# JianCao92/speaker-diarization

Measured on AMD Instinct MI355X. Metric: diarized audio throughput (CD gw/BIC + CL hi/BIC), higher is better.
Workload: dtype f64

## Files before the change

speaker-diarization_amd/csrc/spkd_cluster.hpp:

```cpp
#pragma once
#include "spkd_device.hpp"
#include "spkd_quad.hpp"
#include "spkd_tri.hpp"
#include "../../include/spkd.h"

namespace spkd {

constexpr double MAXINT_F = 9223372036854775808.0;
constexpr double PEN_UNIT = 39.0 + 0.5 * 39.0 * 40.0;
constexpr int AUX = 3 * DA;
constexpr int ERR_DEGENERATE_MERGE = 2;

__device__ __forceinline__ unsigned long long dkey(double v) {
    unsigned long long b = (unsigned long long)__double_as_longlong(v);
    b = (b << 1) ? b : 0ull;
    return (b >> 63) ? ~b : (b | 0x8000000000000000ull);
}
__device__ __forceinline__ double dkey_inv(unsigned long long k) {
    unsigned long long b = (k >> 63) ? (k & 0x7fffffffffffffffull) : ~k;
    return __longlong_as_double((long long)b);
}
template <bool MAXOP>
__device__ __forceinline__ unsigned wave_red_u32(unsigned x) {
    auto op = [](unsigned a, unsigned b) { return MAXOP ? (a > b ? a : b) : (a < b ? a : b); };
// ... 389 lines not shown
    int64_t c = w * 4 + L.m;
    const bool valid = c < n_rec;
    c = valid ? c : n_rec - 1;
    const double* R = qr + c * QREC;
    QuadRows q;
    double sv[QS];
    const double nR = qr_count(R), fR = fast_recip(nR - 1.0);
    quad_load_scaled(R, L.t, fR, q, sv);
    double c1[QS];
    const double gR = -(fR * fast_recip(nR));
#pragma unroll
    for (int s = 0; s < QS; ++s) c1[s] = gR * sv[s];
    TriRank1<0>::run(q, c1, sv);
    auto form_single = [&](int mi, double (&a)[DA]) { single_pair_matrix(kind, recs[mi], recs[mi], true, a); };
    const double v = tri_logdet(q, L.m, err, form_single);
    if (valid && L.t == 0) ld[c] = v;
}

__global__ __launch_bounds__(PT_WAVES * WAVE) void k_cluster_prep(
        const double* __restrict__ qr, int64_t n_rec, int kind,
        double* __restrict__ ld, double* __restrict__ aux, int* err,
        double* pinv_ws) {
    cluster_prep_block(qr, n_rec, kind, ld, aux, err, pinv_ws, blockIdx.x);
}

__global__ __launch_bounds__(PT_WAVES * WAVE) void k_cluster_prep_batch(
        const double* __restrict__ qr, const int64_t* __restrict__ seg_off, int kind,
        double* __restrict__ ld, double* __restrict__ aux, int* prob_err,
        double* pinv_ws) {
    const int64_t off = seg_off[blockIdx.x];
    cluster_prep_block(qr + off * QREC, seg_off[blockIdx.x + 1] - off, kind, ld + off, aux + off * AUX,
                       prob_err + blockIdx.x, pinv_ws, blockIdx.y);
}

__device__ __forceinline__ double finish_distance(int kind, double lambdac, double nA, double ldA,
                                                  double nC, double ldC, double ldx) {
#pragma clang fp contract(off)
    const double n = nA + nC;
    if (kind == SPKD_BIC) {
        double d = 0.5 * n * ldx - 0.5 * nA * ldA - 0.5 * nC * ldC;
        d -= lambdac * 0.5 * PEN_UNIT * log(n);
        return d;
    }
    return -(n / 2.0) * ((nA / n) * ldA + (nC / n) * ldC - ldx);
}

__device__ __forceinline__ int find_problem(const int64_t* __restrict__ seg_off, int64_t n_prob, int64_t g) {
    int64_t lo = 0, hi = n_prob;
    while (hi - lo > 1) {
        int64_t mid = (lo + hi) >> 1;
        if (seg_off[mid] <= g) lo = mid; else hi = mid;
    }
    return (int)lo;
}

#ifndef SPKD_MX_WAVES
#define SPKD_MX_WAVES 4
#endif
constexpr int MX_WAVES = SPKD_MX_WAVES;

template <bool TWO>
__global__ __launch_bounds__(MX_WAVES * WAVE, 2) void k_matrix(
        const double* __restrict__ ex, const double* __restrict__ pk, const int64_t* __restrict__ seg_off,
        const int32_t* __restrict__ rec_prob, const int32_t* __restrict__ sched, int variant, int kind, double lambdac,
        const double* __restrict__ ld, const double* __restrict__ aux,
        double* __restrict__ mat, const int64_t* __restrict__ mat_off,
        unsigned long long* stat_max, unsigned long long* stat_min, int* err) {
    __shared__ double ldsA[QREC];
    const int64_t g = sched[blockIdx.x];
    if (g < 0) return;
    const int p = rec_prob[g];
    const int64_t off = seg_off[p];
    const int64_t N = seg_off[p + 1] - off;
    const int64_t ra = g - off;
    double* Dm = mat + mat_off[p];
    const double* A = ex + g * QREC;
    stage_record(ldsA, A, threadIdx.x, MX_WAVES * WAVE);
    if (variant == 1) {
        if (threadIdx.x == 0) Dm[ra * N + ra] = MAXINT_F;
    } else {
        for (int64_t c = threadIdx.x; c <= ra; c += MX_WAVES * WAVE) Dm[ra * N + c] = __builtin_huge_val();
    }
    __syncthreads();
    const double nA = ldsA[QREC_COUNT_AT];
    const double ldA = ld[g];
    const int wave = threadIdx.x >> 6;
    const QuadLane L = quad_lane();
    if (kind == SPKD_KL2) {
        double wmax = __builtin_nan(""), wmin = __builtin_nan("");
        for (int64_t rc = ra + 1 + wave; rc < N; rc += MX_WAVES) {
            const double d = kl2_from_aux(aux + g * AUX, aux + (off + rc) * AUX);
            if (lane_id() == 0) {
                Dm[ra * N + rc] = d;
                if (variant == 1) Dm[rc * N + ra] = d;
            }
            if (stat_valid(d)) {
                wmax = (wmax != wmax || d > wmax) ? d : wmax;
                wmin = (wmin != wmin || d < wmin) ? d : wmin;
            }
        }
        if (variant == 1 && lane_id() == 0) {
            if (wmax == wmax) atomicMax(stat_max + p, dkey(wmax));
            if (wmin == wmin) atomicMin(stat_min + p, dkey(wmin));
        }
        return;
    }
    double* row = Dm + ra * N;
    for (int64_t base = ra + 1 + 4 * wave; base < N; base += 4 * MX_WAVES) {
        int64_t rc = base + L.m;
        const bool valid = rc < N;
        rc = valid ? rc : N - 1;
        const double det = quad_pair_det<TWO>(kind, ldsA, nA, A, ex + (off + rc) * QREC, pk + (off + rc) * REC, false, L, err);
        if (valid && L.t == 0) row[rc] = det;
    }
    __syncthreads();
    double wmax = __builtin_nan(""), wmin = __builtin_nan("");
    for (int64_t c = ra + 1 + threadIdx.x; c < N; c += MX_WAVES * WAVE) {
        const double det = row[c];
        const double nC = pk[(off + c) * REC + REC - 1];
        const double d = finish_distance(kind, lambdac, nA, ldA, nC, ld[off + c], log(det));
        row[c] = d;
        if (variant == 1) {
            Dm[c * N + ra] = d;
            if (stat_valid(d)) {
                wmax = (wmax != wmax || d > wmax) ? d : wmax;
                wmin = (wmin != wmin || d < wmin) ? d : wmin;
            }
        }
    }
    if (variant == 1) {
        const unsigned long long kmax = wave_red_u64<true>(wmax == wmax ? dkey(wmax) : 0ull);
        const unsigned long long kmin = wave_red_u64<false>(wmin == wmin ? dkey(wmin) : ~0ull);
        if (lane_id() == 0) {
            if (kmax != 0ull) atomicMax(stat_max + p, kmax);
            if (kmin != ~0ull) atomicMin(stat_min + p, kmin);
        }
    }
}

constexpr int AHC_WAVES = 8;
constexpr int AHC_TPB = AHC_WAVES * WAVE;

#ifdef SPKD_PROFILE
__device__ unsigned long long g_step_prof[8];
__device__ unsigned long long g_ahc_prof[8];
constexpr int AHC_SPAN_PROBS = 4096;
__device__ unsigned long long g_ahc_span[2 * AHC_SPAN_PROBS];
#endif
constexpr int NO_COL = 0x7fffffff;
constexpr int AHC_MAX_N = 65536;


struct RowMin { double mv; int mc, nc; };

template <class Alive>
__device__ __forceinline__ RowMin scan_row(const double* __restrict__ row, long long N, Alive alive,
                                           long long sub_col, double sub_val, int lane) {
    double mv = __builtin_huge_val();
    int mc = NO_COL, nc = NO_COL;
    for (long long c0 = 0; c0 < N; c0 += 4 * WAVE) {
        double v[4];
        int a[4];
#pragma unroll
        for (int u = 0; u < 4; ++u) {
            const long long c = c0 + u * WAVE + lane;
            const long long cc = c < N ? c : N - 1;
            a[u] = (c < N) ? (alive(cc) ? 1 : 0) : 0;
            v[u] = row[cc];
        }
#pragma unroll
        for (int u = 0; u < 4; ++u) {
            const long long cl = c0 + u * WAVE + lane;
            const int c = (int)cl;
            if (!a[u]) continue;
            const double x = (cl == sub_col) ? sub_val : v[u];
            if (x != x) { if (c < nc) nc = c; continue; }
            if (x < mv || (x == mv && c < mc)) { mv = x; mc = c; }
        }
    }
    unsigned long long okey;
    unsigned oc;
    wave_argmin_key(mc != NO_COL ? dkey(mv) : ~0ull, (unsigned)mc, okey, oc);
    RowMin r;
    r.mv = okey != ~0ull ? dkey_inv(okey) : __builtin_huge_val();
    r.mc = okey != ~0ull ? (int)oc : NO_COL;
    r.nc = __any(nc != NO_COL) ? (int)wave_red_u32<false>((unsigned)nc) : NO_COL;
    return r;
}

__device__ __forceinline__ bool row_cache_after_merge(int variant, double d, int sa, int sb,
                                                      double& rm, int& ra, int& rn) {
    if (variant != 1) return ra == sb || rn == sb;
    const bool nan_hit = rn == sa || rn == sb;
    if (ra == sa || ra == sb || nan_hit) {
        if (nan_hit || !(d < rm)) return true;
        rm = d; ra = sa;
    } else if (d != d) {
        if (sa < rn) rn = sa;
    } else if (d < rm || (d == rm && sa < ra)) {
        rm = d; ra = sa;
    }
    return false;
}

template <class Alive>
__device__ __forceinline__ double final_matrix_max(const double* __restrict__ Dm, long long N, Alive alive,
                                                   double* s_tmax, int tid) {
    const int lane = tid & (WAVE - 1), wave = tid >> 6;
    double tmax = -__builtin_huge_val();
    bool anynan = false;
    for (long long r = wave; r < N; r += AHC_WAVES) {
        if (!alive(r)) continue;
        const double* row = Dm + r * N;
        for (long long c = lane; c < N; c += WAVE) {
            if (!alive(c)) continue;
            const double v = row[c];
            if (v != v) anynan = true; else tmax = v > tmax ? v : tmax;
        }
    }
#pragma unroll
    for (int s = 1; s < WAVE; s <<= 1) {
        const double t2 = __shfl_xor(tmax, s);
        tmax = t2 > tmax ? t2 : tmax;
    }
    anynan = __any(anynan);
    if (lane == 0) s_tmax[wave] = anynan ? __builtin_nan("") : tmax;
    __syncthreads();
    double mx = s_tmax[0];
    if (tid == 0) {
        for (int w = 1; w < AHC_WAVES; ++w) {
            const double x = s_tmax[w];
            if (mx == mx) mx = (x != x) ? x : (x > mx ? x : mx);
        }
    }
    return mx;
}

__device__ __forceinline__ void refresh_rows(const double* __restrict__ Dm, long long N,
                                             const int32_t* __restrict__ al, int32_t* __restrict__ dirty,
                                             double* __restrict__ rmin, int32_t* __restrict__ rarg,
                                             int32_t* __restrict__ rnan, unsigned long long* masks,
                                             int tid, int wave, int lane) {
    const long long n_chunks = (N + WAVE - 1) / WAVE;
    for (long long ch = wave; ch < n_chunks; ch += AHC_WAVES) {
        const long long rl = ch * WAVE + lane;
        const long long rc = rl < N ? rl : N - 1;
        const int fa = al[rc], fd = dirty[rc];
        const unsigned long long mk = __ballot(rl < N && fa && fd);
        if (lane == 0) masks[ch] = mk;
    }
    __syncthreads();
    int ord = 0;
    for (long long ch = 0; ch < n_chunks; ++ch) {
        const long long r0 = ch * WAVE;
        unsigned long long todo = masks[ch];
        while (todo) {
            const int b = __builtin_ctzll(todo);
            todo &= todo - 1;
            if ((ord++ & (AHC_WAVES - 1)) != wave) continue;
            const long long r = r0 + b;
            const RowMin e = scan_row(Dm + r * N, N, [&](long long c) { return al[c] != 0; }, -1, 0.0, lane);
            if (lane == 0) { rmin[r] = e.mv; rarg[r] = e.mc; rnan[r] = e.nc; dirty[r] = 0; }
#ifdef SPKD_PROFILE
            if (lane == 0) atomicAdd(&g_ahc_prof[0], 1ull);
#endif
        }
    }
}

template <bool TWO>
__global__ __launch_bounds__(AHC_TPB) void k_ahc(
        double* __restrict__ ex, double* __restrict__ pk, const int64_t* __restrict__ seg_off,
        int variant, int kind, int max_spk, double lambdac, double threshold,
        double* __restrict__ ld, double* __restrict__ aux,
        double* __restrict__ mat, const int64_t* __restrict__ mat_off,
        int32_t* __restrict__ alive, double* __restrict__ tmp,
        double* __restrict__ rmin_all, int32_t* __restrict__ rcache_all,
        int32_t* __restrict__ out_n, int32_t* __restrict__ out_a, int32_t* __restrict__ out_b,
        double* __restrict__ out_d, unsigned long long* stat_max, unsigned long long* stat_min,
        double* __restrict__ final_max, double* __restrict__ final_min, int* err,
        double* pinv_ws, const int32_t* __restrict__ prob_of_block) {
    extern __shared__ int32_t ids[];
    __shared__ double ldsA[QREC];
    __shared__ unsigned long long red3[AHC_WAVES][3];
    __shared__ unsigned long long s_masks[AHC_MAX_N / WAVE];
    __shared__ int s_cnt[2];
    __shared__ int s_nids;
    __shared__ int s_next;
    __shared__ double s_tmax[AHC_WAVES];
    const int tid = threadIdx.x, lane = lane_id(), wave = tid >> 6;
    const QuadLane L = quad_lane();
    const int p = prob_of_block ? prob_of_block[blockIdx.x] : (int)blockIdx.x;
#ifdef SPKD_PROFILE
    if (tid == 0 && p < AHC_SPAN_PROBS) g_ahc_span[2 * p] = wall_clock64();
#endif
    const int64_t off = seg_off[p];
    const long long N = seg_off[p + 1] - off;
    double* Dm = mat + mat_off[p];
    int32_t* al = alive + off;
    double* ldp = ld + off;
    double* tp = tmp + off;
    double* rmin = rmin_all + off;
    int32_t* rarg = rcache_all + 3 * off;
    int32_t* rnan = rarg + N;
    int32_t* dirty = rnan + N;
    for (long long c = tid; c < N; c += AHC_TPB) { al[c] = 1; dirty[c] = 1; }
    __syncthreads();
    long long m = N;
    int n_merges = 0;
    const long long INF_IDX = 0x7fffffffffffffffLL;
    double fmin = 0.0;
#ifdef SPKD_PROFILE
    unsigned long long ahc_acc[5] = {0ull, 0ull, 0ull, 0ull, 0ull}, ahc_t = clock64();
#define AHC_TICK(i) do { const unsigned long long now_ = clock64(); ahc_acc[i] += now_ - ahc_t; ahc_t = now_; } while (0)
#else
#define AHC_TICK(i) ((void)0)
#endif
    while (true) {
        refresh_rows(Dm, N, al, dirty, rmin, rarg, rnan, s_masks, tid, wave, lane);
        __syncthreads();
        AHC_TICK(0);
        unsigned long long kb = ~0ull, ib = ~0ull, inan = ~0ull;
        for (long long r = tid; r < N; r += AHC_TPB) {
            if (!al[r]) continue;
            const double v = rmin[r];
            const int c = rarg[r], nc = rnan[r];
            if (nc != NO_COL) { const unsigned long long l = (unsigned long long)(r * N + nc); inan = l < inan ? l : inan; }
            if (c != NO_COL) {
                const unsigned long long kv = dkey(v);
                if (kv < kb) { kb = kv; ib = (unsigned long long)(r * N + c); }
            }
        }
        {
            const unsigned long long wk = wave_red_u64<false>(kb);
            const unsigned long long wi = wave_red_u64<false>(kb == wk ? ib : ~0ull);
            const unsigned long long wn = __any(inan != ~0ull) ? wave_red_u64<false>(inan) : ~0ull;
            if (lane == 0) { red3[wave][0] = wk; red3[wave][1] = wi; red3[wave][2] = wn; }
        }
        __syncthreads();
        unsigned long long bk = red3[0][0], bi = red3[0][1], bn = red3[0][2];
#pragma unroll
        for (int w = 1; w < AHC_WAVES; ++w) {
            const unsigned long long ok = red3[w][0], oi = red3[w][1], on = red3[w][2];
            const bool t = ok < bk || (ok == bk && oi < bi);
            bk = t ? ok : bk; bi = t ? oi : bi;
            bn = on < bn ? on : bn;
        }
        const bool has_nan = bn != ~0ull;
        const double mind = has_nan ? __builtin_nan("") : (bi != ~0ull ? dkey_inv(bk) : __builtin_huge_val());
        const long long index = has_nan ? (long long)bn : (bi != ~0ull ? (long long)bi : INF_IDX);
        fmin = mind;
        const bool go = (mind <= threshold) || (max_spk > 0 && m > max_spk);
        if (!go) break;
        AHC_TICK(1);
        const long long r0 = index / N, c0 = index - r0 * N;
        if (r0 == c0) {
            if (tid == 0) atomicOr(err, ERR_DEGENERATE_MERGE);
            break;
        }
        const long long sa = r0 < c0 ? r0 : c0, sb = r0 < c0 ? c0 : r0;
        if (tid < 2) s_cnt[tid] = 0;
        if (tid == 0) { s_nids = 1; s_next = 0; }
        __syncthreads();
        {
            int ca = 0, cb = 0;
            for (long long c = tid; c < sb; c += AHC_TPB) {
                if (al[c]) { cb++; if (c < sa) ca++; }
            }
            ca = __builtin_amdgcn_readlane(wave_scan_i32(ca), WAVE - 1);
            cb = __builtin_amdgcn_readlane(wave_scan_i32(cb), WAVE - 1);
            if (lane == 0 && ca) atomicAdd(&s_cnt[0], ca);
            if (lane == 0 && cb) atomicAdd(&s_cnt[1], cb);
        }
        __syncthreads();
        if (tid == 0) {
            const int64_t o = off + n_merges;
            out_a[o] = s_cnt[0]; out_b[o] = s_cnt[1]; out_d[o] = mind;
            al[sb] = 0;
            ids[0] = (int32_t)sa;
        }
        n_merges++;
        m--;
#ifdef SPKD_PROFILE
        if (tid == 0) atomicAdd(&g_ahc_prof[1], 1ull);
#endif
        double* A = ex + (off + sa) * QREC;
        const double* B = ex + (off + sb) * QREC;
        {
            double* Ap = pk + (off + sa) * REC;
            const double* Bp = pk + (off + sb) * REC;
            constexpr int NQ = (QREC + AHC_TPB - 1) / AHC_TPB, NP = (REC + AHC_TPB - 1) / AHC_TPB;
            double qa[NQ], qb[NQ], pa[NP], pb[NP];
#pragma unroll
            for (int u = 0; u < NQ; ++u) {
                const int e = tid + u * AHC_TPB;
                qa[u] = A[e < QREC ? e : 0]; qb[u] = B[e < QREC ? e : 0];
            }
#pragma unroll
            for (int u = 0; u < NP; ++u) {
                const int e = tid + u * AHC_TPB;
                pa[u] = Ap[e < REC ? e : 0]; pb[u] = Bp[e < REC ? e : 0];
            }
#pragma unroll
            for (int u = 0; u < NQ; ++u) {
                const int e = tid + u * AHC_TPB;
                const double v = qa[u] + qb[u];
                if (e < QREC) { A[e] = v; ldsA[e] = v; }
            }
#pragma unroll
            for (int u = 0; u < NP; ++u) {
                const int e = tid + u * AHC_TPB;
                if (e < REC) Ap[e] = pa[u] + pb[u];
            }
        }
        __syncthreads();
        for (long long c0 = 0; c0 < N; c0 += AHC_TPB) {
            const long long c = c0 + tid;
            const bool take = c < N && c != sa && al[c < N ? c : N - 1];
            const unsigned long long mk = __ballot(take);
            int base = 0;
            if (lane == 0 && mk) base = atomicAdd(&s_nids, __popcll(mk));
            base = __shfl(base, 0);
            if (take) ids[base + __popcll(mk & ((1ull << lane) - 1ull))] = (int32_t)c;
        }
        __syncthreads();
        AHC_TICK(2);
        const int nids = s_nids;
        const double nA = ldsA[QREC_COUNT_AT];
        if (kind == SPKD_KL2) {
            if (wave == 0) kl2_aux_from_qr(ldsA, aux + (off + sa) * AUX, pinv_ws);
        } else {
            for (;;) {
                int q4 = 0;
                if (lane == 0) q4 = atomicAdd(&s_next, 1);
                const int base = 4 * __builtin_amdgcn_readfirstlane(q4);
                if (base >= nids) break;
                int k = base + L.m;
                const bool valid = k < nids;
                k = valid ? k : nids - 1;
                const int32_t slot = ids[k];
                const double v = quad_pair_det<TWO>(kind, ldsA, nA, A, ex + (off + slot) * QREC, pk + (off + slot) * REC, k == 0, L, err);
                if (valid && L.t == 0) {
                    if (k == 0) ldp[sa] = log(v); else tp[slot] = v;
                }
            }
        }
        __syncthreads();
        AHC_TICK(3);
        double wmax = __builtin_nan(""), wmin = __builtin_nan("");
        const double ldA = ldp[sa];
        for (long long c = tid; c < N; c += AHC_TPB) {
            if (c == sa || !al[c]) continue;
            double d;
            if (kind == SPKD_KL2) {
                d = kl2_from_aux_serial(aux + (off + sa) * AUX, aux + (off + c) * AUX);
            } else {
                const double nC = qr_count(ex + (off + c) * QREC);
                d = finish_distance(kind, lambdac, nA, ldA, nC, ldp[c], log(tp[c]));
            }
            Dm[sa * N + c] = d;
            const double rm0 = rmin[c];
            const int ra0 = rarg[c], rn0 = rnan[c];
            double rm = rm0;
            int ra = ra0, rn = rn0;
            if (variant == 1) Dm[c * N + sa] = d;
            if (row_cache_after_merge(variant, d, (int)sa, (int)sb, rm, ra, rn)) dirty[c] = 1;
            else {
                if (rm != rm0 || ra != ra0) { rmin[c] = rm; rarg[c] = ra; }
                if (rn != rn0) rnan[c] = rn;
            }
            if (variant == 1 && stat_valid(d)) {
                wmax = (wmax != wmax || d > wmax) ? d : wmax;
                wmin = (wmin != wmin || d < wmin) ? d : wmin;
            }
        }
        if (tid == 0) dirty[sa] = 1;
        if (variant == 1) {
            const unsigned long long kmax = wave_red_u64<true>(wmax == wmax ? dkey(wmax) : 0ull);
            const unsigned long long kmin = wave_red_u64<false>(wmin == wmin ? dkey(wmin) : ~0ull);
            if (lane == 0) {
                if (kmax != 0ull) atomicMax(stat_max + p, kmax);
                if (kmin != ~0ull) atomicMin(stat_min + p, kmin);
            }
        }
        __syncthreads();
        AHC_TICK(4);
    }
#ifdef SPKD_PROFILE
    if (tid == 0) for (int i = 0; i < 5; ++i) atomicAdd(&g_ahc_prof[2 + i], ahc_acc[i]);
#endif
    const double mx = final_matrix_max(Dm, N, [&](long long c) { return al[c] != 0; }, s_tmax, tid);
    if (tid == 0) {
        out_n[p] = n_merges;
        final_max[p] = mx;
        final_min[p] = fmin;
#ifdef SPKD_PROFILE
        if (p < AHC_SPAN_PROBS) g_ahc_span[2 * p + 1] = wall_clock64();
#endif
    }
}

constexpr int STEP_WAVES = 4;
constexpr int STEP_WIDE_FROM = 1024;
constexpr int STEP_PARTNERS = 4 * STEP_WAVES - 1;
constexpr int ALIVE_ROUND = 0x7fffffff;
constexpr int STEP_MAX_N = 16384;
constexpr int STEP_IDX_SHIFT = 14;

struct StepState {
    int32_t done, n_merges;
    long long psa;
    double fmin;
    double diag;
};

__host__ __device__ inline unsigned long long step_slot_word(int round, int new_slot, int old_slot) {
    return ((unsigned long long)(unsigned)round << 40) | ((unsigned long long)(unsigned)new_slot << 20) |
           (unsigned long long)(unsigned)old_slot;
}
__device__ __forceinline__ int step_slot_of(unsigned long long w, int k) {
    return ((int)(w >> 40) < k) ? (int)((w >> 20) & 0xfffffull) : (int)(w & 0xfffffull);
}

struct StepSel {
    double rmin, newrow;
    int32_t rarg, rnan, death, pad;
};

struct StepArrays {
    double* ex;
    double* pk;
    double* exm;
    double* pkm;
    int32_t* death;
    StepSel* sel2;
    unsigned long long* sw;
    double* cnt;
    StepState* state2;
    int64_t n_total;
    int32_t n_prob;
};

__global__ __launch_bounds__(AHC_TPB) void k_step_init(
        const int64_t* __restrict__ seg_off, const double* __restrict__ mat,
        const int64_t* __restrict__ mat_off, StepArrays Q) {
    const int lane = lane_id(), wave = threadIdx.x >> 6;
    const int p = blockIdx.y;
    const int64_t off = seg_off[p];
    const long long N = seg_off[p + 1] - off;
    if (blockIdx.x == 0 && threadIdx.x == 0) {
        StepState S;
        S.done = 0; S.n_merges = 0; S.psa = -1; S.fmin = 0.0; S.diag = 0.0;
        Q.state2[(size_t)1 * Q.n_prob + p] = S;
        Q.state2[(size_t)0 * Q.n_prob + p] = S;
    }
    const long long r = (long long)blockIdx.x * AHC_WAVES + wave;
    if (r >= N) return;
    const RowMin m = scan_row(mat + mat_off[p] + r * N, N, [](long long) { return true; }, -1, 0.0, lane);
    if (lane == 0) {
        StepSel e;
        e.rmin = m.mv; e.newrow = 0.0; e.rarg = m.mc; e.rnan = m.nc; e.death = ALIVE_ROUND; e.pad = 0;
        Q.sel2[Q.n_total + off + r] = e;
        Q.sel2[off + r] = e;
        Q.death[off + r] = ALIVE_ROUND;
        Q.sw[off + r] = step_slot_word(0, (int)r, (int)r);
        Q.cnt[off + r] = Q.pk[(off + r) * REC + REC - 1];
    }
}

template <bool TWO, int SW, int SP>
__global__ __launch_bounds__(SW * WAVE) void k_ahc_step(
        int k, const int64_t* __restrict__ seg_off, int variant, int kind, int max_spk, double lambdac,
        double threshold, double* __restrict__ ld, double* __restrict__ aux,
        double* __restrict__ mat, const int64_t* __restrict__ mat_off, StepArrays Q,
        int32_t* __restrict__ out_a, int32_t* __restrict__ out_b, double* __restrict__ out_d,
        unsigned long long* stat_max, unsigned long long* stat_min, int* err,
        double* pinv_ws) {
    constexpr int TPB = SW * WAVE;
    extern __shared__ int32_t s_dyn[];
    __shared__ double ldsA[QREC];
    __shared__ double s_auxA[AUX];
    __shared__ double s_ldx[4 * STEP_WAVES];
    __shared__ double s_dfin[4 * STEP_WAVES];
    __shared__ int s_rescan[4 * STEP_WAVES];
    struct WaveRed { unsigned long long kb, kr, kmax, kmin; unsigned ib, inan; int mc, nc; };
    __shared__ WaveRed wred[SW];
    __shared__ int s_cnt[2];
    const int tid = threadIdx.x, lane = lane_id(), wave = tid >> 6;
    const QuadLane L = quad_lane();
    const int p = blockIdx.y;
#ifdef SPKD_PROFILE
    unsigned long long st_t = clock64();
#define STEP_TICK(i) do { const unsigned long long now_ = clock64(); if (blockIdx.x == 0 && tid == 0) atomicAdd(&g_ahc_prof[i], now_ - st_t); st_t = now_; } while (0)
    unsigned long long st_f = st_t;
#define STEP_FINE(i) do { const unsigned long long now_ = clock64(); if (blockIdx.x == 0 && tid == 0) atomicAdd(&g_step_prof[i], now_ - st_f); st_f = now_; } while (0)
#else
#define STEP_TICK(i) ((void)0)
#define STEP_FINE(i) ((void)0)
#endif
    asm volatile("" :: "s"(Q.state2), "s"(Q.sel2), "s"(Q.sw), "s"(Q.ex), "s"(Q.exm), "s"(Q.n_total), "s"(Q.n_prob),
                 "s"(seg_off), "s"(mat_off), "s"(mat), "s"(k));
    StepState S = Q.state2[(size_t)(k & 1) * Q.n_prob + p];
    StepState* Snext = Q.state2 + (size_t)((k + 1) & 1) * Q.n_prob + p;
    int64_t off = seg_off[p], off_end = seg_off[p + 1], moff = mat_off[p];
    asm volatile("" :: "s"(S.done), "s"(S.n_merges), "s"(off), "s"(off_end), "s"(moff));
    const long long N = off_end - off;
    const bool lead = blockIdx.x == 0;
    if (S.done) {
        if (lead && tid == 0) *Snext = S;
        return;
    }
    STEP_FINE(0);
    const int n_merges = S.n_merges;
    const long long psa = S.psa;
    const long long m = N - n_merges;
    const int n_part = (int)(m - 2);
    constexpr int sp = SP;
    const int nb = n_part > 0 ? (n_part + sp - 1) / sp : 1;
    if ((int)blockIdx.x > nb) return;
    const bool keeper = (int)blockIdx.x == nb;
    int32_t* s_ids = s_dyn;
    int32_t* s_slot = s_dyn + N;
    const int nch = (int)((N + WAVE - 1) / WAVE);
    int32_t* s_base = s_dyn + 2 * N;
    unsigned long long* s_mask = reinterpret_cast<unsigned long long*>(s_dyn + ((2 * N + nch + 1) & ~1LL));
    const int rb = k & 1, wb = (k + 1) & 1;
    const int32_t* death = Q.death + off;
    const StepSel* sel_r = Q.sel2 + (size_t)rb * Q.n_total + off;
    StepSel* sel_w = Q.sel2 + (size_t)wb * Q.n_total + off;
    double* Dm = mat + moff;
    double* ldp = ld + off;
    const long long INF_IDX = 0x7fffffffffffffffLL;
    auto rec_quad = [&](int slot) -> const double* {
        return slot < N ? Q.ex + (off + slot) * QREC : Q.exm + (off + (slot - N)) * QREC;
    };
    auto rec_packed = [&](int slot) -> const double* {
        return slot < N ? Q.pk + (off + slot) * REC : Q.pkm + (off + (slot - N)) * REC;
    };
// ... 474 lines not shown
```

speaker-diarization_amd/csrc/spkd_hip.hip:

```cpp
#include <hip/hip_runtime.h>

#include <algorithm>
#include <cmath>
#include <cstddef>
#include <cstdio>
#include <cstdlib>
#include <cstring>
#include <functional>
#include <string>
#include <atomic>
#include <thread>
#include <vector>

#include "../../include/spkd.h"
#include "spkd_cd.hpp"
#include "spkd_cluster.hpp"
#include "spkd_device.hpp"
#include "spkd_handoff.hpp"
#include "spkd_merge.hpp"
#include "spkd_stats.hpp"
#include "spkd_post_stats.hpp"
#include "spkd_mfcc.hpp"
#include "spkd_mfcc_batch.hpp"
#include "spkd_resample.hpp"
// ... 458 lines not shown
        hipLaunchKernelGGL(k_chunk_stats, dim3((unsigned)chunks.size()), dim3(STATS_TPB), 0, c->stream,
                           d_frames, d_chunks, (double*)d_partial);
    }
    Timer t(c, SPKD_T_REDUCE_SETS);
    hipLaunchKernelGGL(k_reduce_sets, dim3((unsigned)n_sets), dim3(STATS_TPB), 0, c->stream,
                       (const double*)d_partial, d_setoff, d_stats);
    HIPCHK(c, hipGetLastError());
    return SPKD_OK;
}
}

spkd_status spkd_set_stats(spkd_ctx* c, const float* d_frames, int64_t n_frames,
                           const int64_t* h_begin, const int64_t* h_end, const int32_t* h_set,
                           int64_t n_ranges, int64_t n_sets, double* d_stats) {
    if (!c || !d_stats || n_sets < 0 || n_ranges < 0) return SPKD_EINVAL;
    if (n_sets == 0) return SPKD_OK;
    if (n_ranges > 0 && (!h_begin || !h_end || !h_set || !d_frames)) return fail(c, SPKD_EINVAL, "null range arrays");
    std::vector<Chunk> chunks;
    std::vector<int64_t> set_off;
    Call call(c);
    TRY(call.opened);
    TRY(set_stats_launch(c, d_frames, n_frames, h_begin, h_end, h_set, n_ranges, n_sets, d_stats, chunks, set_off));
    return call.finish();
}

spkd_status spkd_pair_terms(spkd_ctx* c, const double* d_stats, const int32_t* h_a, const int32_t* h_b,
                            int64_t n_pairs, int flags, double* h_terms) {
    if (!c || n_pairs < 0) return SPKD_EINVAL;
    if (n_pairs == 0) return SPKD_OK;
    if (!d_stats || !h_a || !h_b || !h_terms) return fail(c, SPKD_EINVAL, "null argument");
    if ((flags & SPKD_WANT_KL2) && (flags & SPKD_WANT_KL2_PINV))
        return fail(c, SPKD_EINVAL, "pair_terms: SPKD_WANT_KL2 and SPKD_WANT_KL2_PINV exclude each other");
    Call call(c);
    TRY(call.opened);
    int kind_unused;
    TRY(use_kind(c, (flags & SPKD_WANT_KL2_PINV) ? (int)SPKD_KL2_PINV : (int)SPKD_KL2, &kind_unused));
    if (flags & SPKD_WANT_KL2_PINV) flags = (flags & ~SPKD_WANT_KL2_PINV) | SPKD_WANT_KL2;
    int32_t *d_a = nullptr, *d_b = nullptr;
    void* d_terms = nullptr;
    TRY(upload(c, S_IDXA, h_a, (size_t)n_pairs, &d_a));
    TRY(upload(c, S_IDXB, h_b, (size_t)n_pairs, &d_b));
    TRY(scratch(c, S_TERMS, (size_t)n_pairs * 8 * sizeof(double), &d_terms));
    const unsigned blocks = (unsigned)((n_pairs + PT2_WAVES - 1) / PT2_WAVES);
    {
        Timer t(c, SPKD_T_PAIR_TERMS);
        hipLaunchKernelGGL(k_pair_terms, dim3(blocks), dim3(PT2_WAVES * WAVE), 0, c->stream,
                           d_stats, d_a, d_b, n_pairs, flags, (double*)d_terms, c->d_err, c->pinv_cur);
    }
    HIPCHK(c, hipGetLastError());
    HIPCHK(c, hipMemcpyAsync(h_terms, d_terms, (size_t)n_pairs * 8 * sizeof(double), hipMemcpyDeviceToHost, c->stream));
    return call.finish();
}

namespace {
struct AhcPrep {
    double* ex;
    double* pk;
    double* ld;
    double* aux;
    double* mat;
    int64_t* seg_off;
    int64_t* mat_off;
    unsigned long long* smax;
    unsigned long long* smin;
    int64_t n_total = 0;
    int64_t grid_rows = 0;
    std::vector<char> offs;
    std::vector<char> prob_of;
    int64_t head_k = 0;
    int64_t grid_head = 0;
    int64_t n_max_head = 0, n_max_rest = 0;
    int32_t *d_prob = nullptr, *d_sched = nullptr, *d_sched_head = nullptr, *d_block_head = nullptr, *d_block_rest = nullptr;
    int variant = 1, kind = 0;
    double lambdac = 0.0;
};

constexpr int N_XCD = 8;
void deal_to_xcds(const int64_t* h_seg_off, const std::vector<int64_t>& order, std::vector<int32_t>& sched,
                  std::vector<int32_t>* by_xcd = nullptr) {
    const int X = N_XCD;
    std::vector<std::vector<int32_t>> lists(X), probs(X);
    if ((int64_t)order.size() >= X) {
        double load[X] = {0, 0, 0, 0, 0, 0, 0, 0};
        for (int64_t p : order) {
            int x = 0;
            for (int i = 1; i < X; ++i) if (load[i] < load[x]) x = i;
            const double n = (double)(h_seg_off[p + 1] - h_seg_off[p]);
            load[x] += n * n;
            probs[x].push_back((int32_t)p);
            for (int64_t r = h_seg_off[p]; r < h_seg_off[p + 1]; ++r) lists[x].push_back((int32_t)r);
        }
    } else {
        std::vector<int64_t> asc(order);
        std::sort(asc.begin(), asc.end());
        int64_t i = 0;
        for (size_t k = 0; k < order.size(); ++k) {
            probs[k].push_back((int32_t)order[k]);
            for (int64_t r = h_seg_off[asc[k]]; r < h_seg_off[asc[k] + 1]; ++r) lists[(size_t)(i++ % X)].push_back((int32_t)r);
        }
    }
    size_t longest = 0;
    for (auto& l : lists) longest = std::max(longest, l.size());
    sched.assign(longest * X, -1);
    for (int x = 0; x < X; ++x)
        for (size_t i = 0; i < lists[x].size(); ++i) sched[i * X + x] = lists[x][i];
    if (by_xcd) {
        by_xcd->clear();
        for (size_t i = 0; by_xcd->size() < order.size(); ++i)
            for (int x = 0; x < X; ++x) if (i < probs[x].size()) by_xcd->push_back(probs[x][i]);
    }
}

unsigned long long host_dkey(double v) {
    unsigned long long b;
    std::memcpy(&b, &v, sizeof b);
    b = (b << 1) ? b : 0ull;
    return (b >> 63) ? ~b : (b | 0x8000000000000000ull);
}

struct MatrixPlan {
    const double* d_init = nullptr;
    double init_max = NAN, init_min = NAN;
    int64_t row_begin = -1, row_end = -1;
    int64_t* d_map = nullptr;
    int64_t n_src = 0;
    const float* d_frames = nullptr;
    int64_t n_frames = 0;
    const int64_t *redo_line = nullptr, *redo_begin = nullptr, *redo_end = nullptr;
    int64_t n_redo = 0;
};

void to_quadrec(spkd_ctx* c, const double* d_stats, int64_t n, double* ex) {
    hipLaunchKernelGGL(k_to_quadrec, dim3((unsigned)n), dim3(256), 0, c->stream, d_stats, n, ex);
}

void cluster_prep(spkd_ctx* c, const double* ex, int64_t n, int kind, double* ld, double* aux) {
    const int64_t per_block = kind == SPKD_KL2 ? PT_WAVES : 4 * PT_WAVES;
    const unsigned blocks = (unsigned)((n + per_block - 1) / per_block);
    hipLaunchKernelGGL(k_cluster_prep, dim3(blocks), dim3(PT_WAVES * WAVE), 0, c->stream, ex, n, kind, ld, aux, c->d_err,
                       c->pinv_cur);
}

void matrix_launch(spkd_ctx* c, const AhcPrep& B, const int32_t* d_sched, int64_t grid) {
    if (grid <= 0) return;
    auto kmat = B.kind == SPKD_GLR ? k_matrix<true> : k_matrix<false>;
    hipLaunchKernelGGL(kmat, dim3((unsigned)grid), dim3(MX_WAVES * WAVE), 0, c->stream,
                       (const double*)B.ex, (const double*)B.pk, (const int64_t*)B.seg_off, (const int32_t*)B.d_prob,
                       d_sched, B.variant, B.kind, B.lambdac,
                       (const double*)B.ld, (const double*)B.aux, B.mat, (const int64_t*)B.mat_off,
                       B.smax, B.smin, c->d_err);
}

constexpr int AHC_HEAD_ROUND = 32;
constexpr double AHC_MS_PER_N2 = 2.122e-4;
constexpr double MATRIX_MS_PER_N2 = 5.58e-7;
constexpr int AHC_HEAD_MAX = 32;
constexpr int AHC_RULE_CUS = 256;
int64_t ahc_head_rule(const std::vector<int64_t>& n, int cus) {
    const int64_t n_prob = (int64_t)n.size();
    if (n_prob < 16) return 0;
    auto t = [](int64_t N) { return AHC_MS_PER_N2 * (double)N * (double)N; };
    double sum_all = 0.0;
    for (int64_t N : n) sum_all += (double)N * (double)N;
    const double stage0 = MATRIX_MS_PER_N2 * sum_all + t(n[0]);
    double best = stage0, sum_head = 0.0;
    int64_t best_k = 0;
    for (int64_t k = 1; k <= std::min<int64_t>(AHC_HEAD_MAX, n_prob) && k < cus; ++k) {
        sum_head += (double)n[(size_t)k - 1] * (double)n[(size_t)k - 1];
        const double m_head = MATRIX_MS_PER_N2 * sum_head, m_rest = MATRIX_MS_PER_N2 * (sum_all - sum_head);
        const double rest = k < n_prob ? m_rest * cus / (double)(cus - k) + t(n[(size_t)k]) : 0.0;
        const double stage = m_head + std::max(t(n[0]), rest);
        if (k % AHC_HEAD_ROUND == 0 && stage < best) { best = stage; best_k = k; }
    }
    return stage0 - best < 0.01 * stage0 ? 0 : best_k;
}

spkd_status ahc_prepare(spkd_ctx* c, const double* d_stats, const int64_t* h_seg_off, int64_t n_prob,
                        int variant, int kind, double lambdac, AhcPrep& B, const MatrixPlan& plan = MatrixPlan()) {
    const int64_t n_total = B.n_total = h_seg_off[n_prob];
    const size_t np = (size_t)n_prob;
    std::vector<int64_t> mat_off(np + 1);
    int64_t cells = 0;
    for (int64_t p = 0; p < n_prob; ++p) {
        const int64_t n = h_seg_off[p + 1] - h_seg_off[p];
        if (n < 0) return fail(c, SPKD_EINVAL, "seg_off must be non-decreasing");
        mat_off[(size_t)p] = cells;
        cells += n * n;
    }
    mat_off[np] = cells;
    std::vector<int32_t> prob((size_t)n_total, 0);
    for (int64_t p = 0; p < n_prob; ++p)
        for (int64_t r = h_seg_off[p]; r < h_seg_off[p + 1]; ++r) prob[(size_t)r] = (int32_t)p;
    {
        std::vector<int32_t> sched, sched_head, block_head, block_rest;
        if (plan.row_begin >= 0) {
            const int64_t rows = plan.row_end - plan.row_begin;
            sched.assign((size_t)((rows + N_XCD - 1) / N_XCD * N_XCD), -1);
            for (int64_t i = 0; i < rows; ++i) sched[(size_t)i] = (int32_t)(plan.row_begin + i);
        } else {
            std::vector<int64_t> order((size_t)n_prob);
            for (int64_t p = 0; p < n_prob; ++p) order[(size_t)p] = p;
            std::stable_sort(order.begin(), order.end(), [&](int64_t a, int64_t b) {
                return h_seg_off[a + 1] - h_seg_off[a] > h_seg_off[b + 1] - h_seg_off[b];
            });
            const std::vector<int64_t> head(order.begin(), order.begin() + B.head_k), rest(order.begin() + B.head_k, order.end());
            deal_to_xcds(h_seg_off, rest, sched);
            if (B.head_k > 0) {
                deal_to_xcds(h_seg_off, head, sched_head, &block_head);
                std::vector<char> in_head((size_t)n_prob, 0);
                for (int64_t p : head) in_head[(size_t)p] = 1;
                for (int64_t p = 0; p < n_prob; ++p) if (!in_head[(size_t)p]) block_rest.push_back((int32_t)p);
                B.n_max_head = h_seg_off[head[0] + 1] - h_seg_off[head[0]];
                B.n_max_rest = rest.empty() ? 0 : h_seg_off[rest[0] + 1] - h_seg_off[rest[0]];
            }
        }
        B.grid_rows = (int64_t)sched.size();
        B.grid_head = (int64_t)sched_head.size();
        TRY(upload_parts(c, S_AHC_OFF, B.offs, [&](Layout L) {
            return L.part(B.seg_off, np + 1, h_seg_off).part(B.mat_off, np + 1, mat_off.data()).bytes();
        }));
        TRY(upload_parts(c, S_AHC_PROB, B.prob_of, [&](Layout L) {
            return L.part(B.d_prob, prob.size(), prob.data()).part(B.d_sched, sched.size(), sched.data())
                .part(B.d_sched_head, sched_head.size(), sched_head.data()).part(B.d_block_head, block_head.size(), block_head.data())
                .part(B.d_block_rest, block_rest.size(), block_rest.data()).bytes();
        }));
    }
    B.variant = variant; B.kind = kind; B.lambdac = lambdac;
    const size_t nt = (size_t)n_total;
    TRY(carve(c, scratch, S_AHC_LD, [&](Layout L) { return L.part(B.ld, nt).bytes(); }));
    TRY(carve(c, scratch, S_AHC_AUX, [&](Layout L) { return L.part(B.aux, nt * AUX).bytes(); }));
    TRY(carve(c, scratch, S_AHC_MAT, [&](Layout L) { return L.part(B.mat, (size_t)cells).bytes(); }));
    TRY(carve(c, scratch, S_AHC_MISC, [&](Layout L) { return L.part(B.smax, np).part(B.smin, np).bytes(); }));
    HIPCHK(c, hipMemsetAsync(B.smax, 0x00, (size_t)n_prob * sizeof(unsigned long long), c->stream));
    HIPCHK(c, hipMemsetAsync(B.smin, 0xff, (size_t)n_prob * sizeof(unsigned long long), c->stream));
    if (plan.d_init && n_prob == 1) {
        c->init_keys[0] = plan.init_max == plan.init_max ? host_dkey(plan.init_max) : 0ull;
        c->init_keys[1] = plan.init_min == plan.init_min ? host_dkey(plan.init_min) : ~0ull;
        HIPCHK(c, hipMemcpyAsync(B.smax, &c->init_keys[0], sizeof(unsigned long long), hipMemcpyHostToDevice, c->stream));
        HIPCHK(c, hipMemcpyAsync(B.smin, &c->init_keys[1], sizeof(unsigned long long), hipMemcpyHostToDevice, c->stream));
    }
    TRY(carve(c, scratch, S_AHC_STATS, [&](Layout L) { return L.part(B.ex, nt * QREC).bytes(); }));
    TRY(carve(c, scratch, S_AHC_PACKED, [&](Layout L) { return L.part(B.pk, nt * REC).bytes(); }));
    if (n_total > 0) {
        if (plan.d_map) {
            void* d_redo = nullptr;
            if (plan.n_redo > 0) {
                int64_t* d_rl = nullptr;
                TRY(scratch(c, S_REDO_STATS, (size_t)plan.n_redo * REC * sizeof(double), &d_redo));
                TRY(upload(c, S_REDO_IDX, plan.redo_line, (size_t)plan.n_redo, &d_rl));
                c->redo_sets.resize((size_t)plan.n_redo);
                for (int64_t k = 0; k < plan.n_redo; ++k) c->redo_sets[(size_t)k] = (int32_t)k;
                TRY(set_stats_launch(c, plan.d_frames, plan.n_frames, plan.redo_begin, plan.redo_end, c->redo_sets.data(),
                                     plan.n_redo, plan.n_redo, (double*)d_redo, c->redo_chunks, c->redo_setoff));
                hipLaunchKernelGGL(k_patch_map, dim3((unsigned)((plan.n_redo + 255) / 256)), dim3(256), 0, c->stream,
                                   (const int64_t*)d_rl, plan.n_redo, plan.d_map);
            }
            hipLaunchKernelGGL(k_records_from_map, dim3((unsigned)n_total), dim3(256), 0, c->stream, d_stats, plan.n_src,
                               (const int64_t*)plan.d_map, (const double*)d_redo, plan.n_redo, n_total, B.ex, B.pk, c->d_err);
        } else {
            to_quadrec(c, d_stats, n_total, B.ex);
            HIPCHK(c, hipMemcpyAsync(B.pk, d_stats, (size_t)n_total * REC * sizeof(double), hipMemcpyDeviceToDevice, c->stream));
        }
        {
            Timer t(c, SPKD_T_CLUSTER_PREP);
            cluster_prep(c, B.ex, n_total, kind, B.ld, B.aux);
        }
        if (plan.d_init) {
            HIPCHK(c, hipMemcpyAsync(B.mat, plan.d_init, (size_t)cells * sizeof(double), hipMemcpyDeviceToDevice, c->stream));
        } else if (B.head_k > 0) {
            (void)hipEventRecord(c->ka[SPKD_T_MATRIX], c->stream);
            matrix_launch(c, B, B.d_sched_head, B.grid_head);
        } else if (B.grid_rows > 0) {
            Timer t(c, SPKD_T_MATRIX);
            matrix_launch(c, B, B.d_sched, B.grid_rows);
        }
    }
    HIPCHK(c, hipGetLastError());
    return SPKD_OK;
}

double key_to_double(unsigned long long k, bool is_max) {
    if (is_max ? (k == 0ull) : (k == ~0ull)) return std::nan("");
    unsigned long long b = (k >> 63) ? (k & 0x7fffffffffffffffull) : ~k;
    double v;
    std::memcpy(&v, &b, sizeof v);
    return v;
}
}

spkd_status spkd_distance_matrix(spkd_ctx* c, int kind, double lambdac, const double* d_stats,
                                 int64_t n, double* d_matrix) {
    if (!c || n < 0 || bad_kind(kind)) return SPKD_EINVAL;
    if (n == 0) return SPKD_OK;
    if (!d_stats || !d_matrix) return fail(c, SPKD_EINVAL, "null argument");
    const int64_t seg_off[2] = {0, n};
    AhcPrep B;
    Call call(c);
    TRY(call.opened);
    TRY(use_kind(c, kind, &kind));
    TRY(ahc_prepare(c, d_stats, seg_off, 1, 1, kind, lambdac, B));
    HIPCHK(c, hipMemcpyAsync(d_matrix, B.mat, (size_t)n * n * sizeof(double), hipMemcpyDeviceToDevice, c->stream));
    return call.finish();
}

spkd_status spkd_cluster_in(spkd_ctx* c, const double* d_stats, int64_t n, int kind, double lambdac, double threshold,
                            int32_t* h_label, double* h_dist, int64_t dist_cap, int64_t* h_dist_off,
                            int64_t* h_n_done, int64_t* h_n_clusters) {
    if (!c || n < 0 || dist_cap < 0 || bad_kind(kind)) return SPKD_EINVAL;
// ... 2564 lines not shown
```

Before: 1580.

## Compute merged row minimum inline and skip refresh when no rows dirty

```diff
diff --git a/speaker-diarization_amd/csrc/spkd_cluster.hpp b/speaker-diarization_amd/csrc/spkd_cluster.hpp
--- a/speaker-diarization_amd/csrc/spkd_cluster.hpp
+++ b/speaker-diarization_amd/csrc/spkd_cluster.hpp
@@ -565,12 +565,36 @@
 
 
 struct RowMin { double mv; int mc, nc; };
+#define ROW_EMPTY RowMin{__builtin_huge_val(), NO_COL, NO_COL}
+
+__device__ __forceinline__ void row_entry_take(RowMin& e, double x, int c) {
+    if (x != x) { if (c < e.nc) e.nc = c; }
+    else if (x < e.mv || (x == e.mv && c < e.mc)) { e.mv = x; e.mc = c; }
+}
+struct RowKey { unsigned long long k; unsigned c, nc; };
+__device__ __forceinline__ RowKey row_entry_wave(const RowMin& e) {
+    RowKey w;
+    wave_argmin_key(e.mc != NO_COL ? dkey(e.mv) : ~0ull, (unsigned)e.mc, w.k, w.c);
+    w.nc = __any(e.nc != NO_COL) ? wave_red_u32<false>((unsigned)e.nc) : (unsigned)NO_COL;
+    return w;
+}
+__device__ __forceinline__ void row_key_meet(RowKey& a, const RowKey& b) {
+    const bool t = b.k < a.k || (b.k == a.k && b.c < a.c);
+    a.k = t ? b.k : a.k; a.c = t ? b.c : a.c;
+    a.nc = b.nc < a.nc ? b.nc : a.nc;
+}
+__device__ __forceinline__ RowMin row_entry_of_key(const RowKey& w) {
+    RowMin r;
+    r.mv = w.k != ~0ull ? dkey_inv(w.k) : __builtin_huge_val();
+    r.mc = w.k != ~0ull ? (int)w.c : NO_COL;
+    r.nc = (int)w.nc;
+    return r;
+}
 
 template <class Alive>
 __device__ __forceinline__ RowMin scan_row(const double* __restrict__ row, long long N, Alive alive,
                                            long long sub_col, double sub_val, int lane) {
-    double mv = __builtin_huge_val();
-    int mc = NO_COL, nc = NO_COL;
+    RowMin e = ROW_EMPTY;
     for (long long c0 = 0; c0 < N; c0 += 4 * WAVE) {
         double v[4];
         int a[4];
@@ -586,19 +610,10 @@
             const long long cl = c0 + u * WAVE + lane;
             const int c = (int)cl;
             if (!a[u]) continue;
-            const double x = (cl == sub_col) ? sub_val : v[u];
-            if (x != x) { if (c < nc) nc = c; continue; }
-            if (x < mv || (x == mv && c < mc)) { mv = x; mc = c; }
-        }
-    }
-    unsigned long long okey;
-    unsigned oc;
-    wave_argmin_key(mc != NO_COL ? dkey(mv) : ~0ull, (unsigned)mc, okey, oc);
-    RowMin r;
-    r.mv = okey != ~0ull ? dkey_inv(okey) : __builtin_huge_val();
-    r.mc = okey != ~0ull ? (int)oc : NO_COL;
-    r.nc = __any(nc != NO_COL) ? (int)wave_red_u32<false>((unsigned)nc) : NO_COL;
-    return r;
+            row_entry_take(e, (cl == sub_col) ? sub_val : v[u], c);
+        }
+    }
+    return row_entry_of_key(row_entry_wave(e));
 }
 
 __device__ __forceinline__ bool row_cache_after_merge(int variant, double d, int sa, int sb,
@@ -608,10 +623,10 @@
     if (ra == sa || ra == sb || nan_hit) {
         if (nan_hit || !(d < rm)) return true;
         rm = d; ra = sa;
-    } else if (d != d) {
-        if (sa < rn) rn = sa;
-    } else if (d < rm || (d == rm && sa < ra)) {
-        rm = d; ra = sa;
+    } else {
+        RowMin e = {rm, ra, rn};
+        row_entry_take(e, d, sa);
+        rm = e.mv; ra = e.mc; rn = e.nc;
     }
     return false;
 }
@@ -701,6 +716,8 @@
     __shared__ int s_nids;
     __shared__ int s_next;
     __shared__ double s_tmax[AHC_WAVES];
+    __shared__ unsigned long long s_own[AHC_WAVES][3];
+    __shared__ int s_ndirty;
     const int tid = threadIdx.x, lane = lane_id(), wave = tid >> 6;
     const QuadLane L = quad_lane();
     const int p = prob_of_block ? prob_of_block[blockIdx.x] : (int)blockIdx.x;
@@ -718,6 +735,7 @@
     int32_t* rnan = rarg + N;
     int32_t* dirty = rnan + N;
     for (long long c = tid; c < N; c += AHC_TPB) { al[c] = 1; dirty[c] = 1; }
+    if (tid == 0) s_ndirty = 1;
     __syncthreads();
     long long m = N;
     int n_merges = 0;
@@ -730,8 +748,10 @@
 #define AHC_TICK(i) ((void)0)
 #endif
     while (true) {
-        refresh_rows(Dm, N, al, dirty, rmin, rarg, rnan, s_masks, tid, wave, lane);
-        __syncthreads();
+        if (s_ndirty != 0) {
+            refresh_rows(Dm, N, al, dirty, rmin, rarg, rnan, s_masks, tid, wave, lane);
+            __syncthreads();
+        }
         AHC_TICK(0);
         unsigned long long kb = ~0ull, ib = ~0ull, inan = ~0ull;
         for (long long r = tid; r < N; r += AHC_TPB) {
@@ -773,70 +793,64 @@
         }
         const long long sa = r0 < c0 ? r0 : c0, sb = r0 < c0 ? c0 : r0;
         if (tid < 2) s_cnt[tid] = 0;
-        if (tid == 0) { s_nids = 1; s_next = 0; }
+        if (tid == 0) { s_nids = 1; s_next = 0; s_ndirty = 0; ids[0] = (int32_t)sa; }
         __syncthreads();
+        double* A = ex + (off + sa) * QREC;
+        const double* B = ex + (off + sb) * QREC;
+        const double diag = Dm[sa * N + sa];
         {
+            double* Ap = pk + (off + sa) * REC;
+            const double* Bp = pk + (off + sb) * REC;
+            constexpr int NQ = (QREC + AHC_TPB - 1) / AHC_TPB, NP = (REC + AHC_TPB - 1) / AHC_TPB;
+            double qa[NQ], qb[NQ], pa[NP], pb[NP];
+#pragma unroll
+            for (int u = 0; u < NQ; ++u) {
+                const int e = tid + u * AHC_TPB;
+                qa[u] = A[e < QREC ? e : 0]; qb[u] = B[e < QREC ? e : 0];
+            }
+#pragma unroll
+            for (int u = 0; u < NP; ++u) {
+                const int e = tid + u * AHC_TPB;
+                pa[u] = Ap[e < REC ? e : 0]; pb[u] = Bp[e < REC ? e : 0];
+            }
             int ca = 0, cb = 0;
-            for (long long c = tid; c < sb; c += AHC_TPB) {
-                if (al[c]) { cb++; if (c < sa) ca++; }
-            }
-            ca = __builtin_amdgcn_readlane(wave_scan_i32(ca), WAVE - 1);
-            cb = __builtin_amdgcn_readlane(wave_scan_i32(cb), WAVE - 1);
+            for (long long c0 = 0; c0 < N; c0 += AHC_TPB) {
+                const long long c = c0 + tid;
+                const bool a = c < N && al[c < N ? c : N - 1];
+                const bool take = a && c != sa && c != sb;
+                ca += __popcll(__ballot(a && c < sa));
+                cb += __popcll(__ballot(a && c < sb));
+                const unsigned long long mk = __ballot(take);
+                int base = 0;
+                if (lane == 0 && mk) base = atomicAdd(&s_nids, __popcll(mk));
+                base = __shfl(base, 0);
+                if (take) ids[base + __popcll(mk & ((1ull << lane) - 1ull))] = (int32_t)c;
+            }
             if (lane == 0 && ca) atomicAdd(&s_cnt[0], ca);
             if (lane == 0 && cb) atomicAdd(&s_cnt[1], cb);
+#pragma unroll
+            for (int u = 0; u < NQ; ++u) {
+                const int e = tid + u * AHC_TPB;
+                const double v = qa[u] + qb[u];
+                if (e < QREC) { A[e] = v; ldsA[e] = v; }
+            }
+#pragma unroll
+            for (int u = 0; u < NP; ++u) {
+                const int e = tid + u * AHC_TPB;
+                if (e < REC) Ap[e] = pa[u] + pb[u];
+            }
         }
         __syncthreads();
         if (tid == 0) {
             const int64_t o = off + n_merges;
             out_a[o] = s_cnt[0]; out_b[o] = s_cnt[1]; out_d[o] = mind;
             al[sb] = 0;
-            ids[0] = (int32_t)sa;
         }
         n_merges++;
         m--;
 #ifdef SPKD_PROFILE
         if (tid == 0) atomicAdd(&g_ahc_prof[1], 1ull);
 #endif
-        double* A = ex + (off + sa) * QREC;
-        const double* B = ex + (off + sb) * QREC;
-        {
-            double* Ap = pk + (off + sa) * REC;
-            const double* Bp = pk + (off + sb) * REC;
-            constexpr int NQ = (QREC + AHC_TPB - 1) / AHC_TPB, NP = (REC + AHC_TPB - 1) / AHC_TPB;
-            double qa[NQ], qb[NQ], pa[NP], pb[NP];
-#pragma unroll
-            for (int u = 0; u < NQ; ++u) {
-                const int e = tid + u * AHC_TPB;
-                qa[u] = A[e < QREC ? e : 0]; qb[u] = B[e < QREC ? e : 0];
-            }
-#pragma unroll
-            for (int u = 0; u < NP; ++u) {
-                const int e = tid + u * AHC_TPB;
-                pa[u] = Ap[e < REC ? e : 0]; pb[u] = Bp[e < REC ? e : 0];
-            }
-#pragma unroll
-            for (int u = 0; u < NQ; ++u) {
-                const int e = tid + u * AHC_TPB;
-                const double v = qa[u] + qb[u];
-                if (e < QREC) { A[e] = v; ldsA[e] = v; }
-            }
-#pragma unroll
-            for (int u = 0; u < NP; ++u) {
-                const int e = tid + u * AHC_TPB;
-                if (e < REC) Ap[e] = pa[u] + pb[u];
-            }
-        }
-        __syncthreads();
-        for (long long c0 = 0; c0 < N; c0 += AHC_TPB) {
-            const long long c = c0 + tid;
-            const bool take = c < N && c != sa && al[c < N ? c : N - 1];
-            const unsigned long long mk = __ballot(take);
-            int base = 0;
-            if (lane == 0 && mk) base = atomicAdd(&s_nids, __popcll(mk));
-            base = __shfl(base, 0);
-            if (take) ids[base + __popcll(mk & ((1ull << lane) - 1ull))] = (int32_t)c;
-        }
-        __syncthreads();
         AHC_TICK(2);
         const int nids = s_nids;
         const double nA = ldsA[QREC_COUNT_AT];
@@ -862,6 +876,7 @@
         AHC_TICK(3);
         double wmax = __builtin_nan(""), wmin = __builtin_nan("");
         const double ldA = ldp[sa];
+        RowMin own = ROW_EMPTY;
         for (long long c = tid; c < N; c += AHC_TPB) {
             if (c == sa || !al[c]) continue;
             double d;
@@ -877,17 +892,24 @@
             double rm = rm0;
             int ra = ra0, rn = rn0;
             if (variant == 1) Dm[c * N + sa] = d;
-            if (row_cache_after_merge(variant, d, (int)sa, (int)sb, rm, ra, rn)) dirty[c] = 1;
-            else {
+            if (row_cache_after_merge(variant, d, (int)sa, (int)sb, rm, ra, rn)) {
+                dirty[c] = 1;
+                atomicAdd(&s_ndirty, 1);
+            } else {
                 if (rm != rm0 || ra != ra0) { rmin[c] = rm; rarg[c] = ra; }
                 if (rn != rn0) rnan[c] = rn;
             }
+            row_entry_take(own, d, (int)c);
             if (variant == 1 && stat_valid(d)) {
                 wmax = (wmax != wmax || d > wmax) ? d : wmax;
                 wmin = (wmin != wmin || d < wmin) ? d : wmin;
             }
         }
-        if (tid == 0) dirty[sa] = 1;
+        {
+            if (tid == (int)(sa % AHC_TPB)) row_entry_take(own, diag, (int)sa);
+            const RowKey w = row_entry_wave(own);
+            if (lane == 0) { s_own[wave][0] = w.k; s_own[wave][1] = w.c; s_own[wave][2] = w.nc; }
+        }
         if (variant == 1) {
             const unsigned long long kmax = wave_red_u64<true>(wmax == wmax ? dkey(wmax) : 0ull);
             const unsigned long long kmin = wave_red_u64<false>(wmin == wmin ? dkey(wmin) : ~0ull);
@@ -897,6 +919,14 @@
             }
         }
         __syncthreads();
+        if (tid == (int)(sa % AHC_TPB)) {
+            RowKey w = {s_own[0][0], (unsigned)s_own[0][1], (unsigned)s_own[0][2]};
+#pragma unroll
+            for (int v = 1; v < AHC_WAVES; ++v)
+                row_key_meet(w, RowKey{s_own[v][0], (unsigned)s_own[v][1], (unsigned)s_own[v][2]});
+            const RowMin e = row_entry_of_key(w);
+            rmin[sa] = e.mv; rarg[sa] = e.mc; rnan[sa] = e.nc;
+        }
         AHC_TICK(4);
     }
 #ifdef SPKD_PROFILE
diff --git a/speaker-diarization_amd/csrc/spkd_hip.hip b/speaker-diarization_amd/csrc/spkd_hip.hip
--- a/speaker-diarization_amd/csrc/spkd_hip.hip
+++ b/speaker-diarization_amd/csrc/spkd_hip.hip
@@ -634,8 +634,8 @@
 }
 
 constexpr int AHC_HEAD_ROUND = 32;
-constexpr double AHC_MS_PER_N2 = 2.122e-4;
-constexpr double MATRIX_MS_PER_N2 = 5.58e-7;
+constexpr double AHC_MS_PER_N2 = 2.054e-4;
+constexpr double MATRIX_MS_PER_N2 = 5.57e-7;
 constexpr int AHC_HEAD_MAX = 32;
 constexpr int AHC_RULE_CUS = 256;
 int64_t ahc_head_rule(const std::vector<int64_t>& n, int cus) {
```

Result: no change. 1590 (median of 6 runs) (+0.6%).
